# WeltXing/PyDyNet

Hardware: AMD Instinct MI355X
Metric: training-step samples/sec (6L Llama3, seq=256) (higher is better)
Workload: dtype f32

## Files before the change

pydynet_amd/csrc/common.h:

```cpp
#pragma once
#include <hip/hip_runtime.h>
#include <stdint.h>
#include <stdio.h>
#include <string.h>

#define PDN_MAX_DIMS 8

enum {
  PDN_OK = 0,
  PDN_EINVAL = -1,
  PDN_EUNSUPPORTED = -2,
  PDN_EWORKSPACE = -3,
};

void pdn_set_error(const char* fmt, ...);

enum {
  PDN_CNT_ROWRES_CHUNK = 0,
  PDN_CNT_ROWTILE_PLAIN = 1,
  PDN_CNT_ROWTILE_SWIGLU_FWD = 2,
  PDN_CNT_ROWTILE_SWIGLU_BWD = 3,
  PDN_CNT_ROWTILE_ROPE = 4,
  PDN_CNT_ROWTILE_ROWMAX = 5,
  PDN_CNT_ROWRES_CHUNK_EPI = 6,
  PDN_CNT_ATT_P_FWD = 7,
  PDN_CNT_ATT_P_BWD = 8,
  PDN_CNT_ATT_RES_FWD = 9,
  PDN_CNT_ATT_RES_BWD = 10,
  PDN_CNT_ATT_STREAM = 11,
  PDN_CNT_CE_DX_DEFERRED = 12,
  PDN_CNT_CE_DW = 13,
  PDN_CNT_OUTRES = 14,
  PDN_CNT_OUTRES_TN = 15,
  PDN_CNT_LINEAR_RELU_FWD = 16,
  PDN_CNT_LINEAR_DX_MASKED = 17,
  PDN_CNT_CE_SMALL = 18,
  PDN_CNT_TILED_SWIGLU_FWD = 19,
  PDN_CNT_TILED_SWIGLU_BWD = 20,
  PDN_CNT_CONV_QUAD_FWD = 21,
  PDN_CNT_CONV_QUAD_DGRAD = 22,
  PDN_CNT_CONV_QUAD_WGRAD = 23,
  PDN_CNT_PATCH_EMBED_FWD = 24,
  PDN_CNT_PATCH_EMBED_BWD = 25,
  PDN_CNT_L2NORM_FWD = 26,
  PDN_CNT_L2NORM_BWD = 27,
  PDN_CNT_SAMPLE = 28,
  PDN_CNT_DECODE_ROWS = 29,
  PDN_CNT_DECODE_SLOTS = 30,
  PDN_CNT_DECODE_WIDE = 31,
  PDN_CNT_BEAM = 32,
  PDN_CNT_EXTEND = 33,
  PDN_CNT_SPECULATE = 34,
  PDN_CNT_PENALTY = 35,
  PDN_CNT_LOGPROBS = 36,
  PDN_CNT_LMHEAD_SPLIT = 37,
  PDN_CNT_PREFIX = 38,
  PDN_CNT_CE_DX_SPLIT = 39,
  PDN_CNT_CE_DW_SPLIT = 40,
  PDN_CNT_ROWTILE_SPLIT = 41,
  PDN_CNT_OUTRES_TN_SPLIT = 42,
  PDN_CNT_ATT_SEG = 43,
  PDN_CNT_ROW_LOSS = 44,
  PDN_CNT_SMOOTH_LOSS = 45,
  PDN_CNT_OUTRES_SPLIT = 46,
  PDN_CNT_PROJ288_SPLIT = 47,
  PDN_CNT_LOGIT_EDIT = 48,
  PDN_CNT_PERSAMPLE = 49,
  PDN_CNT_DOWN_DW_SPLIT = 50,
  PDN_CNT_SLOTS = 51
};
void pdn_count(int slot);

#define PDN_CHECK_ARG(cond, ...)          \
  do {                                    \
    if (!(cond)) {                        \
      pdn_set_error(__VA_ARGS__);         \
      return PDN_EINVAL;                  \
    }                                     \
  } while (0)

#define PDN_LAUNCH_CHECK()                                            \
  do {                                                                \
    hipError_t _e = hipGetLastError();                                \
    if (_e != hipSuccess) {                                           \
      pdn_set_error("%s:%d launch failed: %s", __FILE__, __LINE__,    \
                    hipGetErrorString(_e));                           \
      return (int)_e;                                                 \
    }                                                                 \
  } while (0)

#define PDN_HIP(call)                                                 \
  do {                                                                \
    hipError_t _e = (call);                                           \
    if (_e != hipSuccess) {                                           \
      pdn_set_error("%s:%d %s: %s", __FILE__, __LINE__, #call,        \
                    hipGetErrorString(_e));                           \
      return (int)_e;                                                 \
    }                                                                 \
  } while (0)

static inline int64_t cdiv64(int64_t a, int64_t b) { return (a + b - 1) / b; }

struct PdnView {
  int ndim;
  int64_t shape[PDN_MAX_DIMS];
  int64_t stride[PDN_MAX_DIMS];
};

__device__ __forceinline__ float wave_sum(float v) {
#pragma unroll
  for (int o = 32; o > 0; o >>= 1) v += __shfl_xor(v, o, 64);
  return v;
}
__device__ __forceinline__ float wave_max(float v) {
#pragma unroll
  for (int o = 32; o > 0; o >>= 1) v = fmaxf(v, __shfl_xor(v, o, 64));
  return v;
}
__device__ __forceinline__ double wave_sum(double v) {
#pragma unroll
  for (int o = 32; o > 0; o >>= 1) v += __shfl_xor(v, o, 64);
  return v;
}

template <typename T>
__device__ __forceinline__ T block_sum(T v, T* smem) {
  v = wave_sum(v);
  const int lane = threadIdx.x & 63, wid = threadIdx.x >> 6, nw = (blockDim.x + 63) >> 6;
  if (nw == 1) return v;
  __syncthreads();
  if (lane == 0) smem[wid] = v;
  __syncthreads();
  T r = (T)0;
  for (int i = 0; i < nw; ++i) r += smem[i];
  return r;
}
__device__ __forceinline__ void lds_barrier() {
  asm volatile("s_waitcnt lgkmcnt(0)" ::: "memory");
  __builtin_amdgcn_s_barrier();
  asm volatile("" ::: "memory");
}
__device__ __forceinline__ float block_sum_lds(float v, float* smem) {
  v = wave_sum(v);
  const int lane = threadIdx.x & 63, wid = threadIdx.x >> 6, nw = (blockDim.x + 63) >> 6;
  if (nw == 1) return v;
  lds_barrier();
  if (lane == 0) smem[wid] = v;
  lds_barrier();
  float r = 0.f;
  for (int i = 0; i < nw; ++i) r += smem[i];
  return r;
}
__device__ __forceinline__ float block_max_lds(float v, float* smem) {
  v = wave_max(v);
  const int lane = threadIdx.x & 63, wid = threadIdx.x >> 6, nw = (blockDim.x + 63) >> 6;
  if (nw == 1) return v;
  lds_barrier();
  if (lane == 0) smem[wid] = v;
  lds_barrier();
  float r = smem[0];
  for (int i = 1; i < nw; ++i) r = fmaxf(r, smem[i]);
  return r;
}
__device__ __forceinline__ float block_max(float v, float* smem) {
  v = wave_max(v);
  const int lane = threadIdx.x & 63, wid = threadIdx.x >> 6, nw = (blockDim.x + 63) >> 6;
  if (nw == 1) return v;
  __syncthreads();
  if (lane == 0) smem[wid] = v;
  __syncthreads();
  float r = smem[0];
  for (int i = 1; i < nw; ++i) r = fmaxf(r, smem[i]);
  return r;
}
```

pydynet_amd/csrc/rowtile_split.hip:

```cpp
#include "common.h"
#include "lm_head_split.h"
#include "gemm_rowtile.h"
#include "rowtile_split_index.h"
#include <stdlib.h>
#include <type_traits>

typedef float f32x16 __attribute__((ext_vector_type(16)));
typedef _Float16 f16x8 __attribute__((ext_vector_type(8)));

extern "C" int pdn_malloc(void** ptr, int64_t bytes);
extern "C" int pdn_free(void* ptr);

struct RtsWParams {
  const float* B;
  char* wimg;
  int kind, nper;
  int64_t ldb, bstride;
  unsigned g_off, u_off;
};
__global__ __launch_bounds__(256) void rts_w_kernel(RtsWParams p) {
  __shared__ float sm[RTS_K * 33];
  __shared__ float smax[8 * 32];
  const int tid = threadIdx.x, c = tid & 31, kq = tid >> 5, tile = blockIdx.x;
  float amax = 0.f;
  bool bad = false;
  for (int k = kq; k < RTS_K; k += 8) {
    const float f = p.B[rts_w_src(p.kind, tile, c, k, p.nper, p.ldb, p.bstride, p.g_off, p.u_off)];
    sm[k * 33 + c] = f;
    amax = fmaxf(amax, fabsf(f));
    bad |= !(fabsf(f) < INFINITY);
  }
  smax[kq * 32 + c] = bad ? INFINITY : amax;
  __syncthreads();
  char* img = p.wimg + (int64_t)tile * RTS_TILE;
  float cm = smax[c];
#pragma unroll
  for (int i = 1; i < 8; ++i) cm = fmaxf(cm, smax[i * 32 + c]);
  const int sh = ls_shift(cm);
  for (int u = tid; u < 32 * 36; u += 256) {
    const int ku = u >> 5;
    f16x8 hv, lv;
#pragma unroll
    for (int j = 0; j < 8; ++j) {
      _Float16 h, l;
      ls_split(sm[(8 * ku + j) * 33 + c], sh, h, l);
      hv[j] = h; lv[j] = l;
    }
    char* dst = img + rts_img_unit(c, ku);
    *reinterpret_cast<f16x8*>(dst) = hv;
    *reinterpret_cast<f16x8*>(dst + RTS_PLANE) = lv;
  }
  if (tid < 32) {
    reinterpret_cast<int*>(img + RTS_TAIL)[tid] = -sh;
    reinterpret_cast<float*>(img + RTS_TAIL + 128)[tid] = 0.f;
  }
}

struct RtsParams {
  const float* A;
  int64_t lda;
  const char* wimg;
  float* C;
  float* H;
  unsigned ldc, ldh;
  const float* rope;
  int L, hd, rope_tiles;
  unsigned hd_magic;
  int F;
  const float* norm_w;
  float* xn;
  float* rms;
  int64_t ldxn;
  float norm_eps;
  int M, ntiles, tpw;
  int ablate;
};

template <int V> using rts_ic = std::integral_constant<int, V>;

__device__ __forceinline__ float rts_sigmoid(float g) {
  return __builtin_amdgcn_rcpf(1.f + __builtin_amdgcn_exp2f(-1.4426950408889634f * g));
}

template <int EPI, bool GUARD, bool NORM>
__global__ __launch_bounds__(512, 1) void rts_main_kernel(RtsParams p) {
  static_assert(EPI == 1 || EPI == 3, "SwiGLU or RoPE");
  __shared__ __attribute__((aligned(16))) char smem[RTS_LDS];
  const int tid = threadIdx.x, lane = tid & 63;
  const int wave = __builtin_amdgcn_readfirstlane(tid >> 6);
  const int li = lane & 31, lh = lane >> 5;
  const int m0 = (blockIdx.x * 8 + wave) * 32;
  const int T0 = blockIdx.y * p.tpw;
  const int T1 = min(p.ntiles, T0 + p.tpw);
  if (T0 >= T1) return;

  const bool q4_on = rts_stage_on(4, tid);
  auto stage_ld = [&](const char* base, int q, uint4& r) __attribute__((always_inline)) {
    if (q < 4 || q4_on) r = *reinterpret_cast<const uint4*>(base + (unsigned)rts_stage_unit(q, tid) * 16u);
  };
  auto stage_park = [&](int slot, int q, const uint4& r) __attribute__((always_inline)) {
    if (q < 4 || q4_on) *reinterpret_cast<uint4*>(smem + slot + rts_stage_unit(q, tid) * 16) = r;
  };

  {
    const char* b0 = p.wimg + (int64_t)T0 * RTS_TILE;
    uint4 t0 = make_uint4(0, 0, 0, 0), t1 = t0, t2 = t0, t3 = t0, t4 = t0;
    stage_ld(b0, 0, t0); stage_ld(b0, 1, t1); stage_ld(b0, 2, t2); stage_ld(b0, 3, t3); stage_ld(b0, 4, t4);
    stage_park(0, 0, t0); stage_park(0, 1, t1); stage_park(0, 2, t2); stage_park(0, 3, t3); stage_park(0, 4, t4);
  }
  f16x8 xh[RTS_KS], xl[RTS_KS];
  int nexv = 0;
  if (p.ablate & 2) {
#pragma unroll
    for (int s = 0; s < RTS_KS; ++s)
#pragma unroll
      for (int j = 0; j < 8; ++j) { xh[s][j] = (_Float16)1.f; xl[s][j] = (_Float16)0.5f; }
  } else {
    const char* ap = reinterpret_cast<const char*>(p.A + rts_a_row(m0, li, p.M) * p.lda + rts_a_col(0, lh));
    const char* wp = reinterpret_cast<const char*>(p.norm_w + rts_a_col(0, lh));
    float ss = 0.f, am = 0.f;
    bool bad = false;
#pragma unroll 6
    for (int s = 0; s < RTS_KS; ++s) {
      const float4 a = *reinterpret_cast<const float4*>(ap + 64 * s), b = *reinterpret_cast<const float4*>(ap + 64 * s + 16);
      float4 wa = make_float4(1.f, 1.f, 1.f, 1.f), wb = wa;
      if (NORM) { wa = *reinterpret_cast<const float4*>(wp + 64 * s); wb = *reinterpret_cast<const float4*>(wp + 64 * s + 16); }
      ss += (a.x * a.x + a.y * a.y) + (a.z * a.z + a.w * a.w);
      ss += (b.x * b.x + b.y * b.y) + (b.z * b.z + b.w * b.w);
      const float f0 = fabsf(a.x * wa.x), f1 = fabsf(a.y * wa.y), f2 = fabsf(a.z * wa.z), f3 = fabsf(a.w * wa.w);
      const float f4 = fabsf(b.x * wb.x), f5 = fabsf(b.y * wb.y), f6 = fabsf(b.z * wb.z), f7 = fabsf(b.w * wb.w);
      const float fm = fmaxf(fmaxf(fmaxf(f0, f1), fmaxf(f2, f3)), fmaxf(fmaxf(f4, f5), fmaxf(f6, f7)));
      am = fmaxf(am, fm);
      bad |= !(((f0 + f1) + (f2 + f3)) + ((f4 + f5) + (f6 + f7)) < INFINITY);
    }
    ss += __shfl_xor(ss, 32, 64);
    am = fmaxf(am, __shfl_xor(am, 32, 64));
    bad = bad || (__shfl_xor(bad ? 1 : 0, 32, 64) != 0);
    float inv = 1.f;
    const bool row_w = (!GUARD || m0 + li < p.M) && blockIdx.y == 0 && !(p.ablate & 1);
    if (NORM) {
      const float r = sqrtf(ss / 288.f + p.norm_eps);
      inv = 1.f / r;
      if (lh == 0 && row_w) p.rms[m0 + li] = r;
    }
    const float amax = NORM ? am * inv : am;
    const int sh = ls_shift((bad || !(amax < INFINITY)) ? INFINITY : amax);
    nexv = -sh;
    char* xp = reinterpret_cast<char*>(p.xn + rts_a_row(m0, li, p.M) * p.ldxn + rts_a_col(0, lh));
    asm volatile("" : "+v"(ap));
#pragma unroll
    for (int s0 = 0; s0 < RTS_KS; s0 += 3) {
      float4 xa[3], xb[3], wa[3], wb[3];
#pragma unroll
      for (int e = 0; e < 3; ++e) {
        xa[e] = *reinterpret_cast<const float4*>(ap + 64 * (s0 + e));
        xb[e] = *reinterpret_cast<const float4*>(ap + 64 * (s0 + e) + 16);
        if (NORM) {
          wa[e] = *reinterpret_cast<const float4*>(wp + 64 * (s0 + e));
          wb[e] = *reinterpret_cast<const float4*>(wp + 64 * (s0 + e) + 16);
        }
      }
#pragma unroll
      for (int e = 0; e < 3; ++e) {
        const int s = s0 + e;
        float v[8] = {xa[e].x, xa[e].y, xa[e].z, xa[e].w, xb[e].x, xb[e].y, xb[e].z, xb[e].w};
        if (NORM) {
          const float w[8] = {wa[e].x, wa[e].y, wa[e].z, wa[e].w, wb[e].x, wb[e].y, wb[e].z, wb[e].w};
#pragma unroll
          for (int j = 0; j < 8; ++j) v[j] = v[j] * inv * w[j];
          if (row_w) {
            *reinterpret_cast<float4*>(xp + 64 * s) = make_float4(v[0], v[1], v[2], v[3]);
            *reinterpret_cast<float4*>(xp + 64 * s + 16) = make_float4(v[4], v[5], v[6], v[7]);
          }
        }
#pragma unroll
        for (int j = 0; j < 8; ++j) {
          _Float16 h, l;
          ls_split(v[j], sh, h, l);
          xh[s][j] = h; xl[s][j] = l;
        }
      }
    }
  }

  f32x16 acc0, acc1;
  float out[16];
#pragma unroll
  for (int r = 0; r < 16; ++r) { acc0[r] = 0.f; acc1[r] = 0.f; out[r] = 0.f; }
  const f32x16 zero16 = {0.f, 0.f, 0.f, 0.f, 0.f, 0.f, 0.f, 0.f, 0.f, 0.f, 0.f, 0.f, 0.f, 0.f, 0.f, 0.f};

  const int fr_even = rts_frag_base(li, lh, 0), fr_odd = rts_frag_base(li, lh, 1);
  const int tail_lane = RTS_TAIL + 4 * rts_reg_col(0, lh);
  char* stg = smem + 3 * RTS_TILE + wave * RTS_STG;
  char* stg_w = stg + rts_stg_w(li, lh, 0);
  const char* stg_r = stg + rts_stg_r(lane, 0);
  const char* stgh_r = stg + rts_h_r(lane, 0);
  const bool st_all = !(p.ablate & 1);
  const int srow = m0 + rts_st_row(lane, 0), hrow = m0 + rts_h_row(lane, 0);
  const unsigned ob = 4u * (unsigned)rts_st_row(lane, 0) * p.ldc +
                      (EPI == 1 ? ((lane & 4) ? 4u * (unsigned)p.F + 16u * (unsigned)(lane & 3) : 16u * (unsigned)(lane & 3))
                                : 4u * (unsigned)rts_st_col(lane));
  const unsigned obh = 4u * (unsigned)rts_h_row(lane, 0) * p.ldh + 16u * (unsigned)(lane & 3);
  const unsigned ldc32 = 32u * p.ldc, ldh64 = 64u * p.ldh;
  const unsigned tab_lane = 8u * (unsigned)rts_rope_pos(m0, li, p.L) * (unsigned)p.hd;

  auto rope_ld = [&](int t, int g, float4& r) __attribute__((always_inline)) {
    const unsigned x = 32u * (unsigned)t + 8u * (unsigned)g + 4u * (unsigned)lh;
    const unsigned colh = rts_rope_colh_magic(x, (unsigned)p.hd, p.hd_magic);
    const char* src = reinterpret_cast<const char*>(p.rope) + (tab_lane + 8u * colh);
    const float2 a = *reinterpret_cast<const float2*>(src), b = *reinterpret_cast<const float2*>(src + 16);
    r.x = a.x; r.y = a.y; r.z = b.x; r.w = b.y;
  };
  auto drain_group = [&](int g, const int4& ne, const float4& tb, bool rot) __attribute__((always_inline)) {
    float4 o;
    o.x = ldexpf(out[4 * g + 0], nexv + ne.x);
    o.y = ldexpf(out[4 * g + 1], nexv + ne.y);
    o.z = ldexpf(out[4 * g + 2], nexv + ne.z);
    o.w = ldexpf(out[4 * g + 3], nexv + ne.w);
    if (EPI == 3) {
      const float ex = fmaf(o.x, tb.x, o.y * tb.y), oy = fmaf(o.y, tb.x, -(o.x * tb.y));
      const float ez = fmaf(o.z, tb.z, o.w * tb.w), ow = fmaf(o.w, tb.z, -(o.z * tb.w));
      if (rot) { o.x = ex; o.y = oy; o.z = ez; o.w = ow; }
    }
    *reinterpret_cast<float4*>(__builtin_assume_aligned(stg_w + 32 * g, 16)) = o;
  };
  auto h_group = [&](int g, const int4& ng, const int4& nu) __attribute__((always_inline)) {
    const float g0 = ldexpf(out[4 * g + 0], nexv + ng.x), u0 = ldexpf(out[4 * g + 8], nexv + nu.x);
    const float g1 = ldexpf(out[4 * g + 1], nexv + ng.y), u1 = ldexpf(out[4 * g + 9], nexv + nu.y);
    const float g2 = ldexpf(out[4 * g + 2], nexv + ng.z), u2 = ldexpf(out[4 * g + 10], nexv + nu.z);
    const float g3 = ldexpf(out[4 * g + 3], nexv + ng.w), u3 = ldexpf(out[4 * g + 11], nexv + nu.w);
    float4 o;
    o.x = g0 * rts_sigmoid(g0) * u0; o.y = g1 * rts_sigmoid(g1) * u1;
    o.z = g2 * rts_sigmoid(g2) * u2; o.w = g3 * rts_sigmoid(g3) * u3;
    *reinterpret_cast<float4*>(__builtin_assume_aligned(stg + rts_h_w(li, lh, 0) + 32 * g, 16)) = o;
  };
  auto store_rows = [&](int j, float* Cd) __attribute__((always_inline)) {
    const float4 v = *reinterpret_cast<const float4*>(__builtin_assume_aligned(stg_r + j * (8 * 144), 16));
    if (st_all && (!GUARD || srow + 8 * j < p.M))
      *reinterpret_cast<float4*>(reinterpret_cast<char*>(Cd) + ob + (unsigned)j * ldc32) = v;
  };
  auto store_h = [&](int j, float* Hd) __attribute__((always_inline)) {
    const float4 v = *reinterpret_cast<const float4*>(__builtin_assume_aligned(stgh_r + j * (16 * 144), 16));
    if (st_all && (!GUARD || hrow + 16 * j < p.M))
      *reinterpret_cast<float4*>(reinterpret_cast<char*>(Hd) + obh + (unsigned)j * ldh64) = v;
  };
  auto c_of = [&](int t) -> float* { return p.C + (int64_t)m0 * p.ldc + (EPI == 1 ? 16 : 32) * t; };
  auto h_of = [&](int t) -> float* { return p.H + (int64_t)m0 * p.ldh + 16 * t; };

  auto run_tile = [&](auto firstc, int t, int cur, int prv, int nxt) __attribute__((always_inline)) {
    constexpr bool FIRST = decltype(firstc)::value != 0;
    lds_barrier();
    const char* nb = p.wimg + (int64_t)min(t + 1, T1 - 1) * RTS_TILE;
    float* Cd = c_of(t - 1);
    float* Hd = EPI == 1 ? h_of(t - 1) : nullptr;
    const bool rot = EPI == 3 && t - 1 < p.rope_tiles;
    const char* fe = smem + cur + fr_even;
    const char* fo = smem + cur + fr_odd;
    const char* tl = smem + prv + tail_lane;
    f16x8 wh[2], wl;
    uint4 r0 = make_uint4(0, 0, 0, 0), r1 = r0;
    int4 ne = make_int4(0, 0, 0, 0), nu = ne;
    float4 tb = make_float4(0.f, 0.f, 0.f, 0.f);
#define RTS_LOADH(X, S) wh[X] = *reinterpret_cast<const f16x8*>(__builtin_assume_aligned((((S) & 1) ? fo : fe) + rts_frag_step(S), 16));
#define RTS_LOADL(S) wl = *reinterpret_cast<const f16x8*>(__builtin_assume_aligned((((S) & 1) ? fo : fe) + rts_frag_step(S) + RTS_PLANE, 16));
    RTS_LOADH(0, 0)
    RTS_LOADL(0)
#pragma unroll
    for (int s = 0; s < RTS_KS; ++s) {
      if (s + 1 < RTS_KS) { RTS_LOADH((s + 1) & 1, s + 1) }
      const int dg = EPI == 1 ? (((s & 1) && s < 8) ? (s >> 1) : -1)
                              : (s == 4 ? 0 : s == 8 ? 1 : s == 12 ? 2 : s == 15 ? 3 : -1);
      const int hg = EPI == 1 ? (s == 12 ? 0 : s == 13 ? 1 : -1) : -1;
      if (!FIRST && dg >= 0) ne = *reinterpret_cast<const int4*>(__builtin_assume_aligned(tl + 32 * dg, 16));
      if (!FIRST && hg >= 0) {
        ne = *reinterpret_cast<const int4*>(__builtin_assume_aligned(tl + 32 * hg, 16));
        nu = *reinterpret_cast<const int4*>(__builtin_assume_aligned(tl + 32 * hg + 64, 16));
      }
      __builtin_amdgcn_sched_barrier(0);
      acc0 = __builtin_amdgcn_mfma_f32_32x32x16_f16(wh[s & 1], xh[s], s == 0 ? zero16 : acc0, 0, 0, 0);
      acc1 = __builtin_amdgcn_mfma_f32_32x32x16_f16(wl, xh[s], s == 0 ? zero16 : acc1, 0, 0, 0);
      __builtin_amdgcn_sched_barrier(0);
      if (s + 1 < RTS_KS) { RTS_LOADL(s + 1) }
      acc1 = __builtin_amdgcn_mfma_f32_32x32x16_f16(wh[s & 1], xl[s], acc1, 0, 0, 0);
      __builtin_amdgcn_sched_barrier(0);
      if (s == 6) { stage_park(nxt, 0, r0); stage_park(nxt, 1, r1); }
      if (s == 12) { stage_park(nxt, 2, r0); stage_park(nxt, 3, r1); }
      if (s == 17) stage_park(nxt, 4, r0);
      if (!FIRST && dg >= 0) drain_group(dg, ne, tb, rot);
      if (EPI == 3 && !FIRST && (s == 0 || s == 4 || s == 8 || s == 12)) rope_ld(t - 1, s >> 2, tb);
      if (s == 0) { stage_ld(nb, 0, r0); stage_ld(nb, 1, r1); }
      if (s == 6) { stage_ld(nb, 2, r0); stage_ld(nb, 3, r1); }
      if (s == 12) stage_ld(nb, 4, r0);
      if (EPI == 3 && !FIRST && s >= 16) { store_rows(2 * (s - 16), Cd); store_rows(2 * (s - 16) + 1, Cd); }
      if (EPI == 1 && !FIRST && s >= 8 && s < 12) store_rows(s - 8, Cd);
      if (!FIRST && hg >= 0) h_group(hg, ne, nu);
      if (EPI == 1 && !FIRST && (s == 14 || s == 15)) store_h(s - 14, Hd);
      __builtin_amdgcn_sched_barrier(0);
    }
#undef RTS_LOADH
#undef RTS_LOADL
#pragma unroll
    for (int r = 0; r < 16; ++r) out[r] = fmaf(acc1[r], 1.f / 2048.f, acc0[r]);
  };

  int cur = 0, prv = 2 * RTS_TILE, nxt = RTS_TILE;
  run_tile(rts_ic<1>{}, T0, cur, prv, nxt);
  for (int t = T0 + 1; t < T1; ++t) {
    prv = cur; cur = nxt; nxt = nxt == 2 * RTS_TILE ? 0 : nxt + RTS_TILE;
    run_tile(rts_ic<0>{}, t, cur, prv, nxt);
  }
  {
    float* Cd = c_of(T1 - 1);
    const bool rot = EPI == 3 && T1 - 1 < p.rope_tiles;
    const char* tl = smem + cur + tail_lane;
    float4 tb[4];
#pragma unroll
    for (int g = 0; g < 4; ++g) {
      tb[g] = make_float4(0.f, 0.f, 0.f, 0.f);
      if (EPI == 3) rope_ld(T1 - 1, g, tb[g]);
    }
#pragma unroll
    for (int g = 0; g < 4; ++g) {
      const int4 ne = *reinterpret_cast<const int4*>(__builtin_assume_aligned(tl + 32 * g, 16));
      drain_group(g, ne, tb[g], rot);
    }
    __builtin_amdgcn_sched_barrier(0);
#pragma unroll
    for (int j = 0; j < 4; ++j) store_rows(j, Cd);
    if (EPI == 1) {
      __builtin_amdgcn_sched_barrier(0);
#pragma unroll
      for (int g = 0; g < 2; ++g) {
        const int4 ng = *reinterpret_cast<const int4*>(__builtin_assume_aligned(tl + 32 * g, 16));
        const int4 nu = *reinterpret_cast<const int4*>(__builtin_assume_aligned(tl + 32 * g + 64, 16));
        h_group(g, ng, nu);
      }
      __builtin_amdgcn_sched_barrier(0);
      float* Hd = h_of(T1 - 1);
      store_h(0, Hd); store_h(1, Hd);
    }
  }
}

namespace {
struct RtsTemp {
  void* p = nullptr;
  hipStream_t st = nullptr;
  int get(int64_t bytes, void* stream) { st = (hipStream_t)stream; return pdn_malloc(&p, bytes); }
  ~RtsTemp() {
    static const bool two_stream = getenv("PDN_TWO_STREAM") && atoi(getenv("PDN_TWO_STREAM")) != 0;
    if (p && two_stream) (void)hipStreamSynchronize(st);
    if (p) pdn_free(p);
  }
};
}

static int rts_tiles(const RowTileArgs& a) { return a.epi == 1 ? a.F / 16 : a.N / 32; }

int pdn_rowtile_split_takes(const RowTileArgs& a, void* stream) {
  static const int s_on = ls_env_switch("PDN_ROWTILE_SPLIT", 1, "the q | k | v and gate | up projections stay on the fp32 MFMA kernel");
  if (!s_on || (a.epi != 1 && a.epi != 3) || a.M < RTS_MIN_ROWS || a.b_trans || a.bias || a.residual) return 0;
  if (a.N < 32 || a.N % 32 != 0 || a.nblocks < 1 || (a.N / a.nblocks) * a.nblocks != a.N || (a.N / a.nblocks) % 32 != 0) return 0;
  if ((a.lda & 3) || (a.ldc & 3) || a.lda < RTS_K || a.ldc < a.N || a.ldc >= (1 << 24) || a.ldb < a.N / a.nblocks) return 0;
  if (((uintptr_t)a.A | (uintptr_t)a.C) & 15) return 0;
  if (a.epi == 1 && (a.F < 16 || a.F % 16 != 0 || a.N != 2 * a.F || a.nblocks != 2 || !a.H || (a.ldh & 3) || a.ldh < a.F ||
                     a.ldh >= (1 << 24) || ((uintptr_t)a.H & 15)))
    return 0;
  if (a.epi == 3 && (!a.rope || a.hd < 4 || a.hd % 4 != 0 || a.L < 1 || a.rope_cols % 32 != 0 || a.rope_cols > a.N ||
                     (int64_t)a.L * a.hd >= (1 << 27) || ((uintptr_t)a.rope & 7)))
    return 0;
  if (a.norm_w && !(a.xn && a.rms && (a.ldxn & 3) == 0 && a.ldxn >= RTS_K && (((uintptr_t)a.xn | (uintptr_t)a.norm_w) & 15) == 0)) return 0;
  hipStreamCaptureStatus cs = hipStreamCaptureStatusNone;
  if (hipStreamIsCapturing((hipStream_t)stream, &cs) != hipSuccess) { (void)hipGetLastError(); return 0; }
  return cs == hipStreamCaptureStatusNone ? 1 : 0;
}

int pdn_rowtile_split_launch(const RowTileArgs& a, void* stream) {
  static const int s_ablate = ls_env_switch("PDN_ROWTILE_SPLIT_ABLATE", 0, "timing ablation active, the results of the split q | k | v and gate | up kernels are WRONG");
  const int nt = rts_tiles(a);
  RtsTemp img;
  const int rc = img.get((int64_t)nt * RTS_TILE, stream);
  if (rc) return rc;
  hipStream_t st = (hipStream_t)stream;
  RtsWParams w;
  memset(&w, 0, sizeof(w));
  w.B = a.B; w.wimg = static_cast<char*>(img.p); w.kind = a.epi; w.nper = a.N / a.nblocks; w.ldb = a.ldb;
  w.bstride = a.nblocks > 1 ? a.b_block_stride : 0; w.g_off = a.g_off; w.u_off = a.u_off;
  hipLaunchKernelGGL(rts_w_kernel, dim3(nt), dim3(256), 0, st, w);
  RtsParams p;
  memset(&p, 0, sizeof(p));
  p.A = a.A; p.lda = a.lda; p.wimg = w.wimg; p.C = a.C; p.H = a.H; p.ldc = (unsigned)a.ldc; p.ldh = (unsigned)a.ldh;
  p.rope = a.rope ? a.rope : a.A; p.L = a.L > 0 ? a.L : 1; p.hd = a.hd > 0 ? a.hd : 32; p.rope_tiles = a.rope_cols / 32;
  p.hd_magic = rts_rope_magic(p.hd);
  p.F = a.F; p.norm_w = a.norm_w ? a.norm_w : a.A; p.xn = a.xn ? a.xn : a.C; p.rms = a.rms; p.ldxn = a.ldxn; p.norm_eps = a.norm_eps;
  p.M = a.M; p.ntiles = nt; p.ablate = s_ablate;
  int parts;
  rts_plan(a.M, nt, &p.tpw, &parts);
  const dim3 grid((a.M + 255) / 256, parts), block(512);
  const bool guard = a.M % 256 != 0, norm = a.norm_w != nullptr;
#define RTS_LAUNCH(EPI_)                                                                                      \
  if (guard) { if (norm) hipLaunchKernelGGL((rts_main_kernel<EPI_, true, true>), grid, block, 0, st, p);      \
               else hipLaunchKernelGGL((rts_main_kernel<EPI_, true, false>), grid, block, 0, st, p); }        \
  else { if (norm) hipLaunchKernelGGL((rts_main_kernel<EPI_, false, true>), grid, block, 0, st, p);           \
         else hipLaunchKernelGGL((rts_main_kernel<EPI_, false, false>), grid, block, 0, st, p); }
  if (a.epi == 1) { RTS_LAUNCH(1) } else { RTS_LAUNCH(3) }
#undef RTS_LAUNCH
  pdn_count(PDN_CNT_ROWTILE_PLAIN + a.epi);
  pdn_count(PDN_CNT_ROWTILE_SPLIT);
  PDN_LAUNCH_CHECK();
  return PDN_OK;
}
```

pydynet_amd/csrc/rowtile_split_index.h:

```cpp
#pragma once
#include <stdint.h>

#if defined(__HIPCC__) || defined(__CUDACC__)
#define RTS_HD __host__ __device__ __forceinline__
#else
#define RTS_HD inline
#endif

#define RTS_K 288
#define RTS_KS 18
#define RTS_PLANE (32 * RTS_K * 2)
#define RTS_TAIL (2 * RTS_PLANE)
#define RTS_TILE (RTS_TAIL + 256)
#define RTS_UNITS (RTS_TILE / 16)
#define RTS_STG (32 * 144)
#define RTS_LDS (3 * RTS_TILE + 8 * RTS_STG)
#define RTS_MIN_ROWS 16384

RTS_HD int rts_min_i(int a, int b) { return a < b ? a : b; }

RTS_HD void rts_plan(int64_t M, int ntiles, int* tpw, int* parts) {
  const int64_t row_blocks = (M + 255) / 256;
  int ns = 1;
  while (row_blocks * ns < 256 && ns < ntiles) ++ns;
  const int per = (ntiles + ns - 1) / ns;
  *tpw = per; *parts = (ntiles + per - 1) / per;
}

RTS_HD int64_t rts_w_src(int kind, int tile, int n, int k, int nper, int64_t ldb, int64_t bstride, unsigned g_off, unsigned u_off) {
  if (kind == 1) return (int64_t)(n < 16 ? g_off : u_off) + (int64_t)k * ldb + 16 * tile + (n & 15);
  const int c = 32 * tile + n, b = c / nper;
  return (int64_t)b * bstride + (int64_t)k * ldb + (c - b * nper);
}
RTS_HD int rts_img_unit(int n, int u) { return (n * 36 + (u ^ ((n >> 2) & 3))) * 16; }
RTS_HD int rts_frag_base(int li, int lh, int odd) { return rts_img_unit(li, 2 * odd + lh); }
RTS_HD int rts_frag_step(int s) { return ((2 * s) & ~3) * 16; }
RTS_HD int rts_stage_unit(int q, int tid) { return q * 512 + tid; }
RTS_HD bool rts_stage_on(int q, int tid) { return rts_stage_unit(q, tid) < RTS_UNITS; }

RTS_HD int rts_a_col(int s, int lh) { return 16 * s + 8 * lh; }
RTS_HD int64_t rts_a_row(int64_t m0, int li, int64_t M) { return m0 + li < M ? m0 + li : M - 1; }

RTS_HD int rts_reg_col(int g, int lh) { return 8 * g + 4 * lh; }
RTS_HD int rts_stg_w(int li, int lh, int g) { return li * 144 + 16 * lh + 32 * g; }
RTS_HD int rts_stg_r(int lane, int j) { return ((lane >> 3) + 8 * j) * 144 + (lane & 7) * 16; }
RTS_HD int rts_st_row(int lane, int j) { return (lane >> 3) + 8 * j; }
RTS_HD int rts_st_col(int lane) { return 4 * (lane & 7); }
RTS_HD int rts_out_col(int kind, int tile, int c, int F) { return kind == 1 ? (c < 16 ? 16 * tile + c : F + 16 * tile + c - 16) : 32 * tile + c; }
RTS_HD int rts_h_w(int li, int lh, int g) { return li * 144 + 16 * lh + 32 * g; }
RTS_HD int rts_h_r(int lane, int j) { return ((lane >> 2) + 16 * j) * 144 + (lane & 3) * 16; }
RTS_HD int rts_h_row(int lane, int j) { return (lane >> 2) + 16 * j; }
RTS_HD int rts_h_col(int tile, int lane) { return 16 * tile + 4 * (lane & 3); }

RTS_HD int rts_rope_colh(int tile, int g, int lh, int hd) { return (32 * tile + 8 * g + 4 * lh) % hd; }
RTS_HD unsigned rts_rope_magic(int hd) { return (unsigned)(((1ull << 32) + (unsigned)hd - 1) / (unsigned)hd); }
RTS_HD unsigned rts_rope_colh_magic(unsigned col, unsigned hd, unsigned magic) {
  return col - hd * (unsigned)(((uint64_t)col * magic) >> 32);
}
RTS_HD int rts_rope_pos(int64_t m0, int li, int L) { return (int)((m0 + li) % L); }
RTS_HD int rts_rope_entry(int pos, int colh, int hd) { return (pos * hd + colh) * 2; }
```

Baseline: 9123.

## Route dh + SwiGLU backward through split-fp16 rowtile kernel and coalesce A-row loads

Adds a SwiGLU-backward epilogue (EPI 2) to the split-precision MFMA rowtile kernel. It computes dh = dy·Wᵀ with a transposed weight image, then forms d_gate and d_up in the epilogue from prefetched gate/up values, so the dh backward GEMM leaves the fp32 MFMA path. It also restructures the A-row prologue to use coalesced 8-lane row loads with per-row stats computed by shuffles and staged through LDS. The costs are extra epilogue register pressure and the precision risk of the fp16 split applied to a backward GEMM.

Result: faster. 9339, median of 6 (+2.4%).

```diff
diff --git a/pydynet_amd/csrc/common.h b/pydynet_amd/csrc/common.h
--- a/pydynet_amd/csrc/common.h
+++ b/pydynet_amd/csrc/common.h
@@ -67,7 +67,8 @@
   PDN_CNT_LOGIT_EDIT = 48,
   PDN_CNT_PERSAMPLE = 49,
   PDN_CNT_DOWN_DW_SPLIT = 50,
-  PDN_CNT_SLOTS = 51
+  PDN_CNT_ROWTILE_BWD_SPLIT = 51,
+  PDN_CNT_SLOTS = 52
 };
 void pdn_count(int slot);
 
diff --git a/pydynet_amd/csrc/rowtile_split.hip b/pydynet_amd/csrc/rowtile_split.hip
--- a/pydynet_amd/csrc/rowtile_split.hip
+++ b/pydynet_amd/csrc/rowtile_split.hip
@@ -24,11 +24,24 @@
   const int tid = threadIdx.x, c = tid & 31, kq = tid >> 5, tile = blockIdx.x;
   float amax = 0.f;
   bool bad = false;
-  for (int k = kq; k < RTS_K; k += 8) {
-    const float f = p.B[rts_w_src(p.kind, tile, c, k, p.nper, p.ldb, p.bstride, p.g_off, p.u_off)];
-    sm[k * 33 + c] = f;
-    amax = fmaxf(amax, fabsf(f));
-    bad |= !(fabsf(f) < INFINITY);
+  if (p.kind == 2) {
+    for (int i = tid; i < 32 * RTS_K; i += 256) {
+      const int n = rts_w_t_n(i), k = rts_w_t_k(i);
+      sm[k * 33 + n] = p.B[rts_w_src_t(tile, n, k, p.ldb)];
+    }
+    __syncthreads();
+    for (int k = kq; k < RTS_K; k += 8) {
+      const float f = sm[k * 33 + c];
+      amax = fmaxf(amax, fabsf(f));
+      bad |= !(fabsf(f) < INFINITY);
+    }
+  } else {
+    for (int k = kq; k < RTS_K; k += 8) {
+      const float f = p.B[rts_w_src(p.kind, tile, c, k, p.nper, p.ldb, p.bstride, p.g_off, p.u_off)];
+      sm[k * 33 + c] = f;
+      amax = fmaxf(amax, fabsf(f));
+      bad |= !(fabsf(f) < INFINITY);
+    }
   }
   smax[kq * 32 + c] = bad ? INFINITY : amax;
   __syncthreads();
@@ -62,6 +75,7 @@
   const char* wimg;
   float* C;
   float* H;
+  const float* GU;
   unsigned ldc, ldh;
   const float* rope;
   int L, hd, rope_tiles;
@@ -84,7 +98,8 @@
 
 template <int EPI, bool GUARD, bool NORM>
 __global__ __launch_bounds__(512, 1) void rts_main_kernel(RtsParams p) {
-  static_assert(EPI == 1 || EPI == 3, "SwiGLU or RoPE");
+  static_assert(EPI == 1 || EPI == 2 || EPI == 3, "SwiGLU, SwiGLU backward or RoPE");
+  static_assert(EPI != 2 || !NORM, "SwiGLU backward: no RMSNorm in front");
   __shared__ __attribute__((aligned(16))) char smem[RTS_LDS];
   const int tid = threadIdx.x, lane = tid & 63;
   const int wave = __builtin_amdgcn_readfirstlane(tid >> 6);
@@ -108,6 +123,7 @@
     stage_ld(b0, 0, t0); stage_ld(b0, 1, t1); stage_ld(b0, 2, t2); stage_ld(b0, 3, t3); stage_ld(b0, 4, t4);
     stage_park(0, 0, t0); stage_park(0, 1, t1); stage_park(0, 2, t2); stage_park(0, 3, t3); stage_park(0, 4, t4);
   }
+  char* stg0 = smem + 3 * RTS_TILE + wave * RTS_STG;
   f16x8 xh[RTS_KS], xl[RTS_KS];
   int nexv = 0;
   if (p.ablate & 2) {
@@ -116,63 +132,76 @@
 #pragma unroll
       for (int j = 0; j < 8; ++j) { xh[s][j] = (_Float16)1.f; xl[s][j] = (_Float16)0.5f; }
   } else {
-    const char* ap = reinterpret_cast<const char*>(p.A + rts_a_row(m0, li, p.M) * p.lda + rts_a_col(0, lh));
-    const char* wp = reinterpret_cast<const char*>(p.norm_w + rts_a_col(0, lh));
-    float ss = 0.f, am = 0.f;
-    bool bad = false;
-#pragma unroll 6
-    for (int s = 0; s < RTS_KS; ++s) {
-      const float4 a = *reinterpret_cast<const float4*>(ap + 64 * s), b = *reinterpret_cast<const float4*>(ap + 64 * s + 16);
-      float4 wa = make_float4(1.f, 1.f, 1.f, 1.f), wb = wa;
-      if (NORM) { wa = *reinterpret_cast<const float4*>(wp + 64 * s); wb = *reinterpret_cast<const float4*>(wp + 64 * s + 16); }
-      ss += (a.x * a.x + a.y * a.y) + (a.z * a.z + a.w * a.w);
-      ss += (b.x * b.x + b.y * b.y) + (b.z * b.z + b.w * b.w);
-      const float f0 = fabsf(a.x * wa.x), f1 = fabsf(a.y * wa.y), f2 = fabsf(a.z * wa.z), f3 = fabsf(a.w * wa.w);
-      const float f4 = fabsf(b.x * wb.x), f5 = fabsf(b.y * wb.y), f6 = fabsf(b.z * wb.z), f7 = fabsf(b.w * wb.w);
-      const float fm = fmaxf(fmaxf(fmaxf(f0, f1), fmaxf(f2, f3)), fmaxf(fmaxf(f4, f5), fmaxf(f6, f7)));
-      am = fmaxf(am, fm);
-      bad |= !(((f0 + f1) + (f2 + f3)) + ((f4 + f5) + (f6 + f7)) < INFINITY);
-    }
-    ss += __shfl_xor(ss, 32, 64);
-    am = fmaxf(am, __shfl_xor(am, 32, 64));
-    bad = bad || (__shfl_xor(bad ? 1 : 0, 32, 64) != 0);
-    float inv = 1.f;
-    const bool row_w = (!GUARD || m0 + li < p.M) && blockIdx.y == 0 && !(p.ablate & 1);
-    if (NORM) {
-      const float r = sqrtf(ss / 288.f + p.norm_eps);
-      inv = 1.f / r;
-      if (lh == 0 && row_w) p.rms[m0 + li] = r;
-    }
-    const float amax = NORM ? am * inv : am;
-    const int sh = ls_shift((bad || !(amax < INFINITY)) ? INFINITY : amax);
+    const char* arow[4];
+#pragma unroll
+    for (int i = 0; i < 4; ++i)
+      arow[i] = reinterpret_cast<const char*>(p.A + rts_a_row(m0, rts_pl_row(lane, i), p.M) * p.lda + rts_pl_col(lane, 0));
+    const char* wp = reinterpret_cast<const char*>(p.norm_w + rts_pl_col(lane, 0));
+    float4 xa[RTS_CHUNKS][4];
+#pragma unroll
+    for (int c = 0; c < RTS_CHUNKS; ++c)
+#pragma unroll
+      for (int i = 0; i < 4; ++i) xa[c][i] = *reinterpret_cast<const float4*>(arow[i] + 128 * c);
+    float ss[4] = {0.f, 0.f, 0.f, 0.f}, am[4] = {0.f, 0.f, 0.f, 0.f};
+#pragma unroll
+    for (int c = 0; c < RTS_CHUNKS; ++c) {
+      float4 w = make_float4(1.f, 1.f, 1.f, 1.f);
+      if (NORM) w = *reinterpret_cast<const float4*>(wp + 128 * c);
+#pragma unroll
+      for (int i = 0; i < 4; ++i) {
+        const float4 a = xa[c][i];
+        ss[i] += (a.x * a.x + a.y * a.y) + (a.z * a.z + a.w * a.w);
+        const float f0 = fabsf(a.x * w.x), f1 = fabsf(a.y * w.y), f2 = fabsf(a.z * w.z), f3 = fabsf(a.w * w.w);
+        am[i] = fmaxf(am[i], fmaxf(fmaxf(f0, f1), fmaxf(f2, f3)));
+        if (!((f0 + f1) + (f2 + f3) < INFINITY)) am[i] = INFINITY;
+      }
+    }
+    float inv[4];
+#pragma unroll
+    for (int i = 0; i < 4; ++i) {
+#pragma unroll
+      for (int d = 1; d < 8; d <<= 1) {
+        ss[i] += __shfl_xor(ss[i], d, 64);
+        am[i] = fmaxf(am[i], __shfl_xor(am[i], d, 64));
+      }
+      float r = 1.f;
+      inv[i] = 1.f;
+      if (NORM) { r = sqrtf(ss[i] / 288.f + p.norm_eps); inv[i] = 1.f / r; }
+      const float amax = NORM ? am[i] * inv[i] : am[i];
+      const int sh_i = ls_shift(!(amax < INFINITY) ? INFINITY : amax);
+      if ((lane & 7) == 0)
+        *reinterpret_cast<float2*>(__builtin_assume_aligned(stg0 + rts_pl_stat(rts_pl_row(lane, i)), 8)) = make_float2(r, __int_as_float(sh_i));
+    }
+    const float2 st = *reinterpret_cast<const float2*>(__builtin_assume_aligned(stg0 + rts_pl_stat(li), 8));
+    const int sh = __float_as_int(st.y);
     nexv = -sh;
-    char* xp = reinterpret_cast<char*>(p.xn + rts_a_row(m0, li, p.M) * p.ldxn + rts_a_col(0, lh));
-    asm volatile("" : "+v"(ap));
-#pragma unroll
-    for (int s0 = 0; s0 < RTS_KS; s0 += 3) {
-      float4 xa[3], xb[3], wa[3], wb[3];
-#pragma unroll
-      for (int e = 0; e < 3; ++e) {
-        xa[e] = *reinterpret_cast<const float4*>(ap + 64 * (s0 + e));
-        xb[e] = *reinterpret_cast<const float4*>(ap + 64 * (s0 + e) + 16);
+    const bool wr_on = blockIdx.y == 0 && !(p.ablate & 1);
+    if (NORM && lh == 0 && wr_on && (!GUARD || m0 + li < p.M)) p.rms[m0 + li] = st.x;
+    char* xrow[4];
+#pragma unroll
+    for (int i = 0; i < 4; ++i)
+      xrow[i] = reinterpret_cast<char*>(p.xn + rts_a_row(m0, rts_pl_row(lane, i), p.M) * p.ldxn + rts_pl_col(lane, 0));
+    char* pw = stg0 + rts_pl_stg_w(lane, 0);
+    const char* pf = stg0 + rts_pl_stg_r(li, lh, 0, 0);
+#pragma unroll
+    for (int c = 0; c < RTS_CHUNKS; ++c) {
+      float4 w = make_float4(1.f, 1.f, 1.f, 1.f);
+      if (NORM) w = *reinterpret_cast<const float4*>(wp + 128 * c);
+#pragma unroll
+      for (int i = 0; i < 4; ++i) {
+        float4 v = xa[c][i];
         if (NORM) {
-          wa[e] = *reinterpret_cast<const float4*>(wp + 64 * (s0 + e));
-          wb[e] = *reinterpret_cast<const float4*>(wp + 64 * (s0 + e) + 16);
+          v.x = v.x * inv[i] * w.x; v.y = v.y * inv[i] * w.y; v.z = v.z * inv[i] * w.z; v.w = v.w * inv[i] * w.w;
+          if (wr_on && (!GUARD || m0 + rts_pl_row(lane, i) < p.M)) *reinterpret_cast<float4*>(xrow[i] + 128 * c) = v;
         }
-      }
-#pragma unroll
-      for (int e = 0; e < 3; ++e) {
-        const int s = s0 + e;
-        float v[8] = {xa[e].x, xa[e].y, xa[e].z, xa[e].w, xb[e].x, xb[e].y, xb[e].z, xb[e].w};
-        if (NORM) {
-          const float w[8] = {wa[e].x, wa[e].y, wa[e].z, wa[e].w, wb[e].x, wb[e].y, wb[e].z, wb[e].w};
-#pragma unroll
-          for (int j = 0; j < 8; ++j) v[j] = v[j] * inv * w[j];
-          if (row_w) {
-            *reinterpret_cast<float4*>(xp + 64 * s) = make_float4(v[0], v[1], v[2], v[3]);
-            *reinterpret_cast<float4*>(xp + 64 * s + 16) = make_float4(v[4], v[5], v[6], v[7]);
-          }
-        }
+        *reinterpret_cast<float4*>(__builtin_assume_aligned(pw + i * (8 * 144), 16)) = v;
+      }
+#pragma unroll
+      for (int e = 0; e < 2; ++e) {
+        const int s = 2 * c + e;
+        const float4 va = *reinterpret_cast<const float4*>(__builtin_assume_aligned(pf + 64 * e, 16));
+        const float4 vb = *reinterpret_cast<const float4*>(__builtin_assume_aligned(pf + 64 * e + 16, 16));
+        const float v[8] = {va.x, va.y, va.z, va.w, vb.x, vb.y, vb.z, vb.w};
 #pragma unroll
         for (int j = 0; j < 8; ++j) {
           _Float16 h, l;
@@ -191,7 +220,7 @@
 
   const int fr_even = rts_frag_base(li, lh, 0), fr_odd = rts_frag_base(li, lh, 1);
   const int tail_lane = RTS_TAIL + 4 * rts_reg_col(0, lh);
-  char* stg = smem + 3 * RTS_TILE + wave * RTS_STG;
+  char* stg = stg0;
   char* stg_w = stg + rts_stg_w(li, lh, 0);
   const char* stg_r = stg + rts_stg_r(lane, 0);
   const char* stgh_r = stg + rts_h_r(lane, 0);
@@ -202,6 +231,10 @@
                                 : 4u * (unsigned)rts_st_col(lane));
   const unsigned obh = 4u * (unsigned)rts_h_row(lane, 0) * p.ldh + 16u * (unsigned)(lane & 3);
   const unsigned ldc32 = 32u * p.ldc, ldh64 = 64u * p.ldh;
+  const unsigned Fb = 4u * (unsigned)p.F;
+  const bool gu_on = !(p.ablate & 4);
+  float4 pg[2], pu[2];
+  pg[0] = pg[1] = pu[0] = pu[1] = make_float4(1.f, 1.f, 1.f, 1.f);
   const unsigned tab_lane = 8u * (unsigned)rts_rope_pos(m0, li, p.L) * (unsigned)p.hd;
 
   auto rope_ld = [&](int t, int g, float4& r) __attribute__((always_inline)) {
@@ -244,6 +277,30 @@
     if (st_all && (!GUARD || hrow + 16 * j < p.M))
       *reinterpret_cast<float4*>(reinterpret_cast<char*>(Hd) + obh + (unsigned)j * ldh64) = v;
   };
+  auto gu_ld = [&](int j, const float* Gd, float4& g, float4& u) __attribute__((always_inline)) {
+    if (gu_on && (!GUARD || srow + 8 * j < p.M)) {
+      const char* src = reinterpret_cast<const char*>(Gd) + ob + (unsigned)j * ldc32;
+      g = *reinterpret_cast<const float4*>(src);
+      u = *reinterpret_cast<const float4*>(src + Fb);
+    }
+  };
+  auto store_bwd = [&](int j, float* Cd, const float4& g, const float4& u) __attribute__((always_inline)) {
+    const float4 d = *reinterpret_cast<const float4*>(__builtin_assume_aligned(stg_r + j * (8 * 144), 16));
+    const float dh[4] = {d.x, d.y, d.z, d.w}, gv[4] = {g.x, g.y, g.z, g.w}, uv[4] = {u.x, u.y, u.z, u.w};
+    float dg[4], du[4];
+#pragma unroll
+    for (int i = 0; i < 4; ++i) {
+      const float s = rts_sigmoid(gv[i]), sl = gv[i] * s;
+      const float dsl = fmaf(sl, 1.f - s, s);
+      dg[i] = dh[i] * uv[i] * dsl; du[i] = dh[i] * sl;
+    }
+    if (st_all && (!GUARD || srow + 8 * j < p.M)) {
+      char* dst = reinterpret_cast<char*>(Cd) + ob + (unsigned)j * ldc32;
+      *reinterpret_cast<float4*>(dst) = make_float4(dg[0], dg[1], dg[2], dg[3]);
+      *reinterpret_cast<float4*>(dst + Fb) = make_float4(du[0], du[1], du[2], du[3]);
+    }
+  };
+  auto g_of = [&](int t) -> const float* { return p.GU + (int64_t)m0 * p.ldc + 32 * t; };
   auto c_of = [&](int t) -> float* { return p.C + (int64_t)m0 * p.ldc + (EPI == 1 ? 16 : 32) * t; };
   auto h_of = [&](int t) -> float* { return p.H + (int64_t)m0 * p.ldh + 16 * t; };
 
@@ -269,6 +326,7 @@
     for (int s = 0; s < RTS_KS; ++s) {
       if (s + 1 < RTS_KS) { RTS_LOADH((s + 1) & 1, s + 1) }
       const int dg = EPI == 1 ? (((s & 1) && s < 8) ? (s >> 1) : -1)
+                     : EPI == 2 ? (s < 4 ? s : -1)
                               : (s == 4 ? 0 : s == 8 ? 1 : s == 12 ? 2 : s == 15 ? 3 : -1);
       const int hg = EPI == 1 ? (s == 12 ? 0 : s == 13 ? 1 : -1) : -1;
       if (!FIRST && dg >= 0) ne = *reinterpret_cast<const int4*>(__builtin_assume_aligned(tl + 32 * dg, 16));
@@ -288,9 +346,13 @@
       if (s == 17) stage_park(nxt, 4, r0);
       if (!FIRST && dg >= 0) drain_group(dg, ne, tb, rot);
       if (EPI == 3 && !FIRST && (s == 0 || s == 4 || s == 8 || s == 12)) rope_ld(t - 1, s >> 2, tb);
+      if (EPI == 2 && !FIRST && (s == 4 || s == 5)) store_bwd(s - 4, Cd, pg[s - 4], pu[s - 4]);
+      if (EPI == 2 && !FIRST && s == 6) { gu_ld(2, g_of(t - 1), pg[0], pu[0]); gu_ld(3, g_of(t - 1), pg[1], pu[1]); }
+      if (EPI == 2 && !FIRST && (s == 11 || s == 12)) store_bwd(s - 9, Cd, pg[s - 11], pu[s - 11]);
       if (s == 0) { stage_ld(nb, 0, r0); stage_ld(nb, 1, r1); }
       if (s == 6) { stage_ld(nb, 2, r0); stage_ld(nb, 3, r1); }
       if (s == 12) stage_ld(nb, 4, r0);
+      if (EPI == 2 && s == 13) { gu_ld(0, g_of(t), pg[0], pu[0]); gu_ld(1, g_of(t), pg[1], pu[1]); }
       if (EPI == 3 && !FIRST && s >= 16) { store_rows(2 * (s - 16), Cd); store_rows(2 * (s - 16) + 1, Cd); }
       if (EPI == 1 && !FIRST && s >= 8 && s < 12) store_rows(s - 8, Cd);
       if (!FIRST && hg >= 0) h_group(hg, ne, nu);
@@ -319,14 +381,22 @@
       tb[g] = make_float4(0.f, 0.f, 0.f, 0.f);
       if (EPI == 3) rope_ld(T1 - 1, g, tb[g]);
     }
+    float4 lg[2], lu[2];
+    lg[0] = lg[1] = lu[0] = lu[1] = make_float4(1.f, 1.f, 1.f, 1.f);
+    if (EPI == 2) { gu_ld(2, g_of(T1 - 1), lg[0], lu[0]); gu_ld(3, g_of(T1 - 1), lg[1], lu[1]); }
 #pragma unroll
     for (int g = 0; g < 4; ++g) {
       const int4 ne = *reinterpret_cast<const int4*>(__builtin_assume_aligned(tl + 32 * g, 16));
       drain_group(g, ne, tb[g], rot);
     }
     __builtin_amdgcn_sched_barrier(0);
-#pragma unroll
-    for (int j = 0; j < 4; ++j) store_rows(j, Cd);
+    if (EPI == 2) {
+      store_bwd(0, Cd, pg[0], pu[0]); store_bwd(1, Cd, pg[1], pu[1]);
+      store_bwd(2, Cd, lg[0], lu[0]); store_bwd(3, Cd, lg[1], lu[1]);
+    } else {
+#pragma unroll
+      for (int j = 0; j < 4; ++j) store_rows(j, Cd);
+    }
     if (EPI == 1) {
       __builtin_amdgcn_sched_barrier(0);
 #pragma unroll
@@ -358,14 +428,21 @@
 static int rts_tiles(const RowTileArgs& a) { return a.epi == 1 ? a.F / 16 : a.N / 32; }
 
 int pdn_rowtile_split_takes(const RowTileArgs& a, void* stream) {
-  static const int s_on = ls_env_switch("PDN_ROWTILE_SPLIT", 1, "the q | k | v and gate | up projections stay on the fp32 MFMA kernel");
-  if (!s_on || (a.epi != 1 && a.epi != 3) || a.M < RTS_MIN_ROWS || a.b_trans || a.bias || a.residual) return 0;
+  static const int s_on = ls_env_switch("PDN_ROWTILE_SPLIT", 1, "the q | k | v and gate | up projections and dh + SwiGLU backward stay on the fp32 MFMA kernel");
+  if (!s_on || (a.epi != 1 && a.epi != 2 && a.epi != 3) || a.M < RTS_MIN_ROWS || a.bias || a.residual) return 0;
+  if ((a.epi == 2) != (a.b_trans != 0)) return 0;
   if (a.N < 32 || a.N % 32 != 0 || a.nblocks < 1 || (a.N / a.nblocks) * a.nblocks != a.N || (a.N / a.nblocks) % 32 != 0) return 0;
-  if ((a.lda & 3) || (a.ldc & 3) || a.lda < RTS_K || a.ldc < a.N || a.ldc >= (1 << 24) || a.ldb < a.N / a.nblocks) return 0;
+  if ((a.lda & 3) || (a.ldc & 3) || a.lda < RTS_K || a.ldc < a.N || a.ldc >= (1 << 24) || a.ldb < (a.b_trans ? RTS_K : a.N / a.nblocks)) return 0;
   if (((uintptr_t)a.A | (uintptr_t)a.C) & 15) return 0;
   if (a.epi == 1 && (a.F < 16 || a.F % 16 != 0 || a.N != 2 * a.F || a.nblocks != 2 || !a.H || (a.ldh & 3) || a.ldh < a.F ||
                      a.ldh >= (1 << 24) || ((uintptr_t)a.H & 15)))
     return 0;
+  if (a.epi == 2) {
+    if (a.F < 32 || a.F % 32 != 0 || a.N != a.F || a.nblocks != 1 || a.ldc < 2 * (int64_t)a.F || !a.GU || ((uintptr_t)a.GU & 15)) return 0;
+    const float* ce = a.C + (int64_t)a.M * a.ldc;
+    if ((const float*)a.C < a.GU + (int64_t)a.M * a.ldc && a.GU < ce) return 0;
+    if ((const float*)a.C < a.A + (int64_t)a.M * a.lda && a.A < ce) return 0;
+  }
   if (a.epi == 3 && (!a.rope || a.hd < 4 || a.hd % 4 != 0 || a.L < 1 || a.rope_cols % 32 != 0 || a.rope_cols > a.N ||
                      (int64_t)a.L * a.hd >= (1 << 27) || ((uintptr_t)a.rope & 7)))
     return 0;
@@ -376,7 +453,7 @@
 }
 
 int pdn_rowtile_split_launch(const RowTileArgs& a, void* stream) {
-  static const int s_ablate = ls_env_switch("PDN_ROWTILE_SPLIT_ABLATE", 0, "timing ablation active, the results of the split q | k | v and gate | up kernels are WRONG");
+  static const int s_ablate = ls_env_switch("PDN_ROWTILE_SPLIT_ABLATE", 0, "timing ablation active, the results of the split q | k | v, gate | up and dh + SwiGLU backward kernels are WRONG");
   const int nt = rts_tiles(a);
   RtsTemp img;
   const int rc = img.get((int64_t)nt * RTS_TILE, stream);
@@ -389,7 +466,7 @@
   hipLaunchKernelGGL(rts_w_kernel, dim3(nt), dim3(256), 0, st, w);
   RtsParams p;
   memset(&p, 0, sizeof(p));
-  p.A = a.A; p.lda = a.lda; p.wimg = w.wimg; p.C = a.C; p.H = a.H; p.ldc = (unsigned)a.ldc; p.ldh = (unsigned)a.ldh;
+  p.A = a.A; p.lda = a.lda; p.wimg = w.wimg; p.C = a.C; p.H = a.H; p.GU = a.GU ? a.GU : a.A; p.ldc = (unsigned)a.ldc; p.ldh = (unsigned)a.ldh;
   p.rope = a.rope ? a.rope : a.A; p.L = a.L > 0 ? a.L : 1; p.hd = a.hd > 0 ? a.hd : 32; p.rope_tiles = a.rope_cols / 32;
   p.hd_magic = rts_rope_magic(p.hd);
   p.F = a.F; p.norm_w = a.norm_w ? a.norm_w : a.A; p.xn = a.xn ? a.xn : a.C; p.rms = a.rms; p.ldxn = a.ldxn; p.norm_eps = a.norm_eps;
@@ -403,10 +480,13 @@
                else hipLaunchKernelGGL((rts_main_kernel<EPI_, true, false>), grid, block, 0, st, p); }        \
   else { if (norm) hipLaunchKernelGGL((rts_main_kernel<EPI_, false, true>), grid, block, 0, st, p);           \
          else hipLaunchKernelGGL((rts_main_kernel<EPI_, false, false>), grid, block, 0, st, p); }
-  if (a.epi == 1) { RTS_LAUNCH(1) } else { RTS_LAUNCH(3) }
+  if (a.epi == 1) { RTS_LAUNCH(1) }
+  else if (a.epi == 3) { RTS_LAUNCH(3) }
+  else if (guard) hipLaunchKernelGGL((rts_main_kernel<2, true, false>), grid, block, 0, st, p);
+  else hipLaunchKernelGGL((rts_main_kernel<2, false, false>), grid, block, 0, st, p);
 #undef RTS_LAUNCH
   pdn_count(PDN_CNT_ROWTILE_PLAIN + a.epi);
-  pdn_count(PDN_CNT_ROWTILE_SPLIT);
+  pdn_count(a.epi == 2 ? PDN_CNT_ROWTILE_BWD_SPLIT : PDN_CNT_ROWTILE_SPLIT);
   PDN_LAUNCH_CHECK();
   return PDN_OK;
 }
diff --git a/pydynet_amd/csrc/rowtile_split_index.h b/pydynet_amd/csrc/rowtile_split_index.h
--- a/pydynet_amd/csrc/rowtile_split_index.h
+++ b/pydynet_amd/csrc/rowtile_split_index.h
@@ -32,6 +32,9 @@
   const int c = 32 * tile + n, b = c / nper;
   return (int64_t)b * bstride + (int64_t)k * ldb + (c - b * nper);
 }
+RTS_HD int64_t rts_w_src_t(int tile, int n, int k, int64_t ldb) { return (int64_t)(32 * tile + n) * ldb + k; }
+RTS_HD int rts_w_t_n(int i) { return i / RTS_K; }
+RTS_HD int rts_w_t_k(int i) { return i % RTS_K; }
 RTS_HD int rts_img_unit(int n, int u) { return (n * 36 + (u ^ ((n >> 2) & 3))) * 16; }
 RTS_HD int rts_frag_base(int li, int lh, int odd) { return rts_img_unit(li, 2 * odd + lh); }
 RTS_HD int rts_frag_step(int s) { return ((2 * s) & ~3) * 16; }
@@ -41,12 +44,21 @@
 RTS_HD int rts_a_col(int s, int lh) { return 16 * s + 8 * lh; }
 RTS_HD int64_t rts_a_row(int64_t m0, int li, int64_t M) { return m0 + li < M ? m0 + li : M - 1; }
 
+#define RTS_CHUNKS 9
+RTS_HD int rts_pl_row(int lane, int i) { return (lane >> 3) + 8 * i; }
+RTS_HD int rts_pl_col(int lane, int c) { return 32 * c + 4 * (lane & 7); }
+RTS_HD int rts_pl_stat(int row) { return row * 16; }
+RTS_HD int rts_pl_stg_w(int lane, int i) { return rts_pl_row(lane, i) * 144 + (lane & 7) * 16; }
+RTS_HD int rts_pl_stg_r(int li, int lh, int e, int half) { return li * 144 + 64 * e + 32 * lh + 16 * half; }
+
 RTS_HD int rts_reg_col(int g, int lh) { return 8 * g + 4 * lh; }
 RTS_HD int rts_stg_w(int li, int lh, int g) { return li * 144 + 16 * lh + 32 * g; }
 RTS_HD int rts_stg_r(int lane, int j) { return ((lane >> 3) + 8 * j) * 144 + (lane & 7) * 16; }
 RTS_HD int rts_st_row(int lane, int j) { return (lane >> 3) + 8 * j; }
 RTS_HD int rts_st_col(int lane) { return 4 * (lane & 7); }
 RTS_HD int rts_out_col(int kind, int tile, int c, int F) { return kind == 1 ? (c < 16 ? 16 * tile + c : F + 16 * tile + c - 16) : 32 * tile + c; }
+RTS_HD int rts_bwd_gate_col(int tile, int c) { return 32 * tile + c; }
+RTS_HD int rts_bwd_up_col(int tile, int c, int F) { return F + 32 * tile + c; }
 RTS_HD int rts_h_w(int li, int lh, int g) { return li * 144 + 16 * lh + 32 * g; }
 RTS_HD int rts_h_r(int lane, int j) { return ((lane >> 2) + 16 * j) * 144 + (lane & 3) * 16; }
 RTS_HD int rts_h_row(int lane, int j) { return (lane >> 2) + 16 * j; }
```
